# CloudResolvingClimateModeling/sp-coupler

Measured on AMD Instinct MI355X. Metric: SP column-exchanges/sec (GCM<->LES forcing+tendency), higher is better.
Workload: dtype f64

## Files before the change

include/spc.h:

```cpp
#ifndef SPC_H
#define SPC_H

#include <stdint.h>

#ifdef __cplusplus
extern "C" {
#endif

#define SPC_ABI_VERSION 4

typedef enum spc_status {
    SPC_OK = 0,
    SPC_ERR_INVALID_ARGUMENT = -1,
    SPC_ERR_UNSUPPORTED = -2,
    SPC_ERR_LAUNCH = -3,
    SPC_ERR_NO_DEVICE = -4
} spc_status;

typedef struct spc_dims {
    int64_t n_cols;
    int32_t nG;
    int32_t nL;
    int64_t pitchG;
    int64_t pitchGh;
    int64_t pitchL;
    int32_t les_grid_shared;
    int32_t cols_per_block;
} spc_dims;

typedef struct spc_forward_args {
    const void *U, *V, *T, *SH, *QL, *QI, *Pf;
    const void *Ph;
    const void *Zgfull;
    const void *Zghalf;
    const void *zf;
    const void *zh;
    const void *u_d, *v_d, *thl_d, *qt_d, *ql_d;
    const void *ps_d;
    const void *rain, *rain_last;
    double factor;
    double dt;
    void *f_u, *f_v, *f_thl, *f_qt, *f_ql, *ql_ref;
    void *f_ps;
    void *u, *v, *thl, *qt;
    void *ps;
    void *Zf;
    void *Zh;
    void *rainrate;
    int32_t *idx;
    const void *Z0M, *Z0H, *QLflux, *QIflux, *SHflux, *TSflux;
    void *z0m, *z0h, *wthl, *wqt;
} spc_forward_args;

int spc_forward_f64(const spc_dims *dims, const spc_forward_args *args, void *stream);
int spc_forward_f32(const spc_dims *dims, const spc_forward_args *args, void *stream);

int spc_cloud_indices_f64(const spc_dims *dims, const void *zh, const void *Zh, int32_t *idx, void *stream);
int spc_cloud_indices_f32(const spc_dims *dims, const void *zh, const void *Zh, int32_t *idx, void *stream);

typedef struct spc_backward_args {
    const void *T, *SH, *QL, *QI, *U, *V, *A;
    const void *Zf;
    const void *Zgfull, *Zghalf;
    const void *zf;
    const void *t_d, *qt_d, *ql_d, *ql_ice_d, *u_d, *v_d;
    const void *A_prof;
    const void *zh;
    const void *Zh;
    const void *rhobf_d;
    int32_t conservative;
    int32_t reserved;
    double factor;
    double dt;
    void *f_T, *f_SH, *f_QL, *f_QI, *f_U, *f_V, *f_A;
    int32_t *start_index;
} spc_backward_args;

int spc_backward_f64(const spc_dims *dims, const spc_backward_args *args, void *stream);
int spc_backward_f32(const spc_dims *dims, const spc_backward_args *args, void *stream);

typedef struct spc_diagnostics_args {
    const void *T, *SH, *QL, *QI, *Pf;
    const void *Zgfull, *Zghalf;
    const void *zf;
    const void *thl_d, *ql_d, *ql_ice_d;
    void *Tv, *THL, *QT;
    void *Zf;
    void *Zh;
    void *pf, *t, *ql_water;
} spc_diagnostics_args;

int spc_diagnostics_f64(const spc_dims *dims, const spc_diagnostics_args *args, void *stream);
int spc_diagnostics_f32(const spc_dims *dims, const spc_diagnostics_args *args, void *stream);

int spc_surface_fluxes_f64(int64_t n, const void *Ph_s, const void *T_s, const void *QLflux, const void *QIflux,
                           const void *SHflux, const void *TSflux, void *wthl, void *wqt, void *stream);
int spc_surface_fluxes_f32(int64_t n, const void *Ph_s, const void *T_s, const void *QLflux, const void *QIflux,
                           const void *SHflux, const void *TSflux, void *wthl, void *wqt, void *stream);

typedef struct spc_vnudge_args {
    int64_t n_cols;
    int32_t itot, jtot, ktot;
    int32_t constantT;
    void *qt;
// ... 179 lines not shown
```

sp_coupler_amd/_abi.py:

```python
import ctypes
import os

ABI_VERSION = 4
_HERE = os.path.dirname(os.path.abspath(__file__))
LIB_NAME = "libspc_hip.so"
LIB_PATH = os.path.join(_HERE, LIB_NAME)

c_void_p, c_double, c_int32, c_int64 = ctypes.c_void_p, ctypes.c_double, ctypes.c_int32, ctypes.c_int64
c_int32_p = ctypes.POINTER(ctypes.c_int32)

SPC_OK, SPC_ERR_INVALID_ARGUMENT, SPC_ERR_UNSUPPORTED, SPC_ERR_LAUNCH, SPC_ERR_NO_DEVICE = 0, -1, -2, -3, -4


class SpcError(RuntimeError):

    def __init__(self, code, text):
        super().__init__("spc error %d: %s" % (code, text))
        self.code = code


class SpcInvalidArgument(SpcError, ValueError):
    pass


class SpcLibraryError(ImportError):
    """The HIP extension is missing or does not match include/spc.h."""


class Dims(ctypes.Structure):
    _fields_ = [("n_cols", c_int64), ("nG", c_int32), ("nL", c_int32), ("pitchG", c_int64),
                ("pitchGh", c_int64), ("pitchL", c_int64), ("les_grid_shared", c_int32),
                ("cols_per_block", c_int32)]


def _ptrs(*names):
    return [(n, c_void_p) for n in names]


class ForwardArgs(ctypes.Structure):
    _fields_ = (_ptrs("U", "V", "T", "SH", "QL", "QI", "Pf", "Ph", "Zgfull", "Zghalf", "zf", "zh",
                      "u_d", "v_d", "thl_d", "qt_d", "ql_d", "ps_d", "rain", "rain_last")
                + [("factor", c_double), ("dt", c_double)]
                + _ptrs("f_u", "f_v", "f_thl", "f_qt", "f_ql", "ql_ref", "f_ps", "u", "v", "thl", "qt", "ps",
                        "Zf", "Zh", "rainrate", "idx", "Z0M", "Z0H", "QLflux", "QIflux", "SHflux", "TSflux",
                        "z0m", "z0h", "wthl", "wqt"))


class BackwardArgs(ctypes.Structure):
    _fields_ = (_ptrs("T", "SH", "QL", "QI", "U", "V", "A", "Zf", "Zgfull", "Zghalf", "zf",
                      "t_d", "qt_d", "ql_d", "ql_ice_d", "u_d", "v_d", "A_prof", "zh", "Zh", "rhobf_d")
                + [("conservative", c_int32), ("reserved", c_int32), ("factor", c_double), ("dt", c_double)]
                + _ptrs("f_T", "f_SH", "f_QL", "f_QI", "f_U", "f_V", "f_A", "start_index"))


class DiagnosticsArgs(ctypes.Structure):
    _fields_ = _ptrs("T", "SH", "QL", "QI", "Pf", "Zgfull", "Zghalf", "zf", "thl_d", "ql_d", "ql_ice_d",
                     "Tv", "THL", "QT", "Zf", "Zh", "pf", "t", "ql_water")


class VnudgeArgs(ctypes.Structure):
    _fields_ = ([("n_cols", c_int64), ("itot", c_int32), ("jtot", c_int32), ("ktot", c_int32), ("constantT", c_int32)]
                + _ptrs("qt", "qsat", "thl", "ql", "R", "ql_av", "qt_av", "presf", "ql_ref", "beta", "a_add", "qt_std", "status", "work")
                + [("work_bytes", c_int64)])


class InterpArgs(ctypes.Structure):
    _fields_ = ([("n_rows", c_int64), ("n_x", c_int32), ("n_xp", c_int32), ("pitch_x", c_int64), ("pitch_xp", c_int64),
                 ("pitch_fp", c_int64), ("pitch_out", c_int64)] + _ptrs("x", "xp", "fp", "out"))


class SearchsortedArgs(ctypes.Structure):
    _fields_ = ([("n_rows", c_int64), ("n_a", c_int32), ("n_v", c_int32), ("pitch_a", c_int64), ("pitch_v", c_int64),
                 ("pitch_out", c_int64)] + _ptrs("a", "v", "out") + [("side_right", c_int32), ("reserved", c_int32)])


class InterpCArgs(ctypes.Structure):
    _fields_ = ([("n_rows", c_int64), ("nG", c_int32), ("nL", c_int32), ("pitch_Zh", c_int64), ("pitch_zh", c_int64),
                 ("pitch_q", c_int64), ("pitch_out", c_int64)] + _ptrs("Zh", "zh", "q", "rho", "out")
                + [("mode", c_int32), ("reserved", c_int32)])


class PipArgs(ctypes.Structure):
    _fields_ = ([("n_points", c_int64), ("n_vertices", c_int64), ("n_rings", c_int32), ("n_polys", c_int32)]
                + _ptrs("lon", "lat", "vx", "vy", "ring_start", "ring_role", "ring_poly", "out"))


class LesStateArgs(ctypes.Structure):
    _fields_ = ([("n_les", c_int64)] + _ptrs("elem_off", "ktot") + [("prof", c_void_p * 4), ("pitch_prof", c_int64),
                ("amp", c_double * 4), ("out", c_void_p * 4)] + _ptrs("key_in") + [("pos_in", c_int32), ("reserved", c_int32)]
                + _ptrs("key_out", "pos_out") + [("gens_per_substream", c_int64)] + _ptrs("work") + [("work_bytes", c_int64)])


SLAB_MAX_FIELDS = 16


class SlabMeansArgs(ctypes.Structure):
    _fields_ = [("n_les", c_int64), ("itot", c_int32), ("jtot", c_int32), ("ktot", c_int32), ("n_fields", c_int32),
                ("fields", c_void_p * SLAB_MAX_FIELDS), ("out", c_void_p * SLAB_MAX_FIELDS), ("pitch_out", c_int64)]
# ... 152 lines not shown
```

sp_coupler_amd/csrc/spc_device.hpp:

```cpp
#pragma once

constexpr int BLOCK = 256;
constexpr int MAX_LDS_BYTES = 64 * 1024;
constexpr int HARD_LDS_BYTES = 160 * 1024;

template <typename T> struct K {
    static constexpr T pref0 = T(1e5), rd = T(287.04), rv = T(461.5), cp = T(1004.), rlv = T(2.53e6),
                       grav = T(9.81);
};

#define SPC_POW_FN __device__ __forceinline__
#include "spc_pow.h"
__device__ __forceinline__ double spc_pow_special(double x, double y)
{
    if (x != x) return x;
    const double big = __builtin_huge_val();
    if (x == 0.0) return y < 0.0 ? big : 0.0;
    if (x == big || x == -big) return y < 0.0 ? 0.0 : big;
    return __builtin_nan("");
}
__device__ __forceinline__ double spc_pow(double x, double y)
{
    if (!(x > 0.0 && x <= 1.7976931348623157e308)) return spc_pow_special(x, y);
    return spc_pow_pos(x, y);
// ... 209 lines not shown
    while (lo < hi) {
        const int mid = lo + ((hi - lo) >> 1);
        if (z[mid] < a) lo = mid + 1; else hi = mid;
    }
    return lo - 1;
}

__host__ __device__ inline int su_pad(int p2) { return 2 * p2 + 2; }

template <int SL, typename T, typename Pred> __device__ __forceinline__ const T *su_seek(const T *row, int p2, const Pred &adv)
{
    const T *p = row;
    if constexpr (SL > 0) {
#pragma unroll
        for (int s = 1 << (SL - 1); s > 0; s >>= 1) {
            const T *const nx = p + s;
            p = adv(p[s - 1]) ? nx : p;
        }
    } else {
        for (int s = p2; s > 0; s >>= 1) {
            const T *const nx = p + s;
            p = adv(p[s - 1]) ? nx : p;
        }
    }
    return p;
}

template <int SL, typename T, typename Pred> __device__ __forceinline__ int su_count(const T *row, int p2, const Pred &adv)
{
    return (int)(((unsigned)(size_t)su_seek<SL>(row, p2, adv) - (unsigned)(size_t)row) / (unsigned)sizeof(T));
}

struct DimsP {
    int64_t n_cols, pitchG, pitchGh, pitchL;
    int nG, nL, cb, p2G, p2L, shared_grid, xcd_remap;
};

struct Empty {};

template <typename T> struct FwdOpt {
    const T *rain, *rain_last;
    T *u, *v, *thl, *qt, *ps, *Zf, *Zh, *rainrate;
    const T *Z0M, *Z0H, *QLflux, *QIflux, *SHflux, *TSflux;
    T *z0m, *z0h, *wthl, *wqt;
};

template <typename T, bool FULL> struct FwdP {
    DimsP d;
    const T *U, *V, *Tm, *SH, *QL, *QI, *Pf, *Ph, *Zgfull, *Zghalf, *zf, *zh;
    const T *u_d, *v_d, *thl_d, *qt_d, *ql_d, *ps_d;
    T factor, dt;
    T *f_u, *f_v, *f_thl, *f_qt, *f_ql, *ql_ref, *f_ps;
    int32_t *idx;
    typename std::conditional<FULL, FwdOpt<T>, Empty>::type o;
};

template <typename T> using FwdFull = FwdP<T, true>;

template <typename T> struct BwdP {
    DimsP d;
    const T *Tm, *SH, *QL, *QI, *U, *V, *A, *Zf, *Zgfull, *Zghalf, *zf;
    const T *t_d, *qt_d, *ql_d, *ql_ice_d, *u_d, *v_d, *A_prof;
    const T *zh, *Zh, *rhobf_d;
    T factor, dt;
    T *f_T, *f_SH, *f_QL, *f_QI, *f_U, *f_V, *f_A;
    int32_t *start_index;
};

template <typename T> struct DiagP {
    DimsP d;
    const T *Tm, *SH, *QL, *QI, *Pf, *Zgfull, *Zghalf, *zf, *thl_d, *ql_d, *ql_ice_d;
    T *Tv, *THL, *QT, *Zf, *Zh, *pf, *t, *ql_water;
};

extern __shared__ __align__(16) unsigned char spc_smem[];

__device__ __forceinline__ unsigned slab_index(int remap)
{
    if (remap) {
        const unsigned b = blockIdx.x, nb = gridDim.x, x = b & 7u, j = b >> 3, q = nb >> 3, r = nb & 7u;
        return x * q + (x < r ? x : r) + j;
    }
    return blockIdx.x;
}

#ifdef SPC_STAMPS
__device__ unsigned long long *g_stamps = nullptr;
#define STAMP(i)                                                                     \
    do {                                                                             \
        if (threadIdx.x == 0 && g_stamps && (SPC_STAMPS == 1 || (i) == 0 || (i) == 5)) {  \
            asm volatile("s_waitcnt vmcnt(0) lgkmcnt(0)" ::: "memory");              \
            g_stamps[(size_t)blockIdx.x * 8 + (i)] = wall_clock64();                 \
        }                                                                            \
    } while (0)
#else
#define STAMP(i) do { } while (0)
#endif
```

sp_coupler_amd/csrc/spc_k1.hpp:

```cpp
#pragma once

template <typename T> struct LesIn {
    T h, ud, vd, thld, qtd, qld;
};

template <typename P, typename T = decltype(+*P().zf)>
__device__ __forceinline__ LesIn<T> load_les(const P &p, int l, int64_t o)
{
    LesIn<T> r;
    r.h = p.d.shared_grid ? ldg(&p.zf[l]) : ldg(&p.zf[o]);
    r.ud = ldg(&p.u_d[o]); r.vd = ldg(&p.v_d[o]); r.thld = ldg(&p.thl_d[o]); r.qtd = ldg(&p.qt_d[o]); r.qld = ldg(&p.ql_d[o]);
    return r;
}

constexpr int cfloor_pow2(int n) { int p = 1; while (p * 2 <= n) p *= 2; return p; }

template <typename T, bool FULL, int NG, int NL, int WT, int BLK = BLOCK, bool PRE = true>
__global__ __launch_bounds__(BLK) void k_forward(const FwdP<T, FULL> p)
{
    const DimsP &d = p.d;
#define OPT(f) (*(decltype(FwdOpt<T>::f) const volatile __attribute__((address_space(4))) *)( \
    (const char __attribute__((address_space(4))) *)__builtin_amdgcn_kernarg_segment_ptr() + offsetof(FwdFull<T>, o) + offsetof(FwdOpt<T>, f)))
    const int nG = NG ? NG : d.nG, nL = NL ? NL : d.nL, cb = d.cb;
    const int64_t pitchG = NG ? NG : d.pitchG, pitchGh = NG ? NG + 1 : d.pitchGh, pitchL = NL ? NL : d.pitchL;
    const int p2G = NG ? cfloor_pow2(NG ? NG : 1) : d.p2G;
    const int tid = threadIdx.x;
    const int64_t col0 = (int64_t)slab_index(d.xcd_remap) * cb;
    const int ncol = (int)((d.n_cols - col0) < cb ? (d.n_cols - col0) : cb);
    T *const lds = reinterpret_cast<T *>(spc_smem);
    T *const lzh = lds + (size_t)cb * 6 * nG;
    const int n1 = ncol * nG, n2 = ncol * nL, nI = p.idx ? n1 : 0, nitems = n2 + nI;
    constexpr bool REACH = !PRE;
    STAMP(0);

    LesIn<T> pre2 = {};
    T pre_zgh = T(0), pre_zs = T(0);
    if (!PRE) {
    } else if (tid < n2) {
        const int c = tid / nL, l = tid - c * nL;
        pre2 = load_les<FwdP<T, FULL>, T>(p, l, (col0 + c) * pitchL + l);
    } else if (tid < nitems) {
        const int ei = tid - n2, c = ei / nG, m = ei - c * nG;
        const int64_t gh = (col0 + c) * pitchGh;
        pre_zgh = ldg(&p.Zghalf[gh + (nG - 1 - m)]);
        pre_zs = ldg(&p.Zghalf[gh + nG]);
    }
    const int sc = BLK - 1 - tid;
    T sc_ps = T(0), sc_psd = T(0), sc_rain = T(0), sc_rl = T(0);
    if (PRE && sc < ncol) {
        sc_ps = ldg(&p.Ph[(col0 + sc) * pitchGh + nG]);
        sc_psd = ldg(&p.ps_d[col0 + sc]);
        if constexpr (FULL)
            if (OPT(rainrate)) { sc_rain = OPT(rain)[col0 + sc]; sc_rl = OPT(rain_last)[col0 + sc]; }
    }
    if (p.idx) {
        const int nz = d.shared_grid ? nL : n2;
        for (int e = tid; e < nz; e += BLK) {
            const int c = e / nL, l = e - c * nL;
            lzh[e] = d.shared_grid ? p.zh[e] : p.zh[(col0 + c) * pitchL + l];
        }
    }
    STAMP(1);

    int nR = nG;
    if constexpr (REACH) {
        __shared__ T s_wmax[BLK / 64];
        __shared__ int s_top;
        if (tid == 0) s_top = 0;
        for (int e = tid; e < n1; e += BLK) {
            const int c = e / nG, k = e - c * nG;
            const int64_t col = col0 + c, g = col * pitchG + k;
            const T zf_k = div_grav(ldg(&p.Zgfull[g]) - ldg(&p.Zghalf[col * pitchGh + nG]));
            lds[(size_t)c * 6 * nG + (nG - 1 - k)] = zf_k;
            if constexpr (FULL)
                if (OPT(Zf)) OPT(Zf)[g] = zf_k;
        }
        T hmax = T(-__builtin_huge_val());
        for (int e = tid, nz = d.shared_grid ? nL : n2; e < nz; e += BLK) {
            const int c = e / nL, l = e - c * nL;
            const T h = d.shared_grid ? ldg(&p.zf[e]) : ldg(&p.zf[(col0 + c) * pitchL + l]);
            hmax = h > hmax ? h : hmax;
        }
        for (int m = 32; m > 0; m >>= 1) {
            const T o = __shfl_xor(hmax, m, 64);
            hmax = o > hmax ? o : hmax;
        }
        if ((tid & 63) == 0) s_wmax[tid >> 6] = hmax;
        __syncthreads();
        if (tid < ncol) {
            for (int w = 0; w < BLK / 64; ++w) hmax = s_wmax[w] > hmax ? s_wmax[w] : hmax;
            const Br<T> b = bracket2(lds + (size_t)tid * 6 * nG, nG, p2G, hmax);
            atomicMax(&s_top, b.j0 + 1 >= nG ? nG - 1 : b.j0 + 1);
        }
        __syncthreads();
        nR = s_top + 1;
    }
    const float rcp_nR = 1.0f / (float)nR;
    for (int e = tid; e < ncol * nR; e += BLK) {
        int c, k;
        if constexpr (REACH) {
            c = (int)((float)e * rcp_nR);
            int r = e - c * nR;
            if (r < 0) { --c; r += nR; } else if (r >= nR) { ++c; r -= nR; }
            k = nG - nR + r;
        } else {
            c = e / nG; k = e - c * nG;
        }
        const int64_t col = col0 + c, g = col * pitchG + k;
        const T zsurf = REACH ? T(0) : ldg(&p.Zghalf[col * pitchGh + nG]);
        const T tt = ldg(&p.Tm[g]), sh = ldg(&p.SH[g]), ql = ldg(&p.QL[g]), qi = ldg(&p.QI[g]), pf = ldg(&p.Pf[g]);
        const T zg = REACH ? T(0) : ldg(&p.Zgfull[g]);
        const T uu = ldg(&p.U[g]), vv = ldg(&p.V[g]);
        T *const s = lds + (size_t)c * 6 * nG + (nG - 1 - k);
        if constexpr (!REACH) {
            const T zf_k = div_grav(zg - zsurf);
            s[0] = zf_k;
            if constexpr (FULL)
                if (OPT(Zf)) OPT(Zf)[g] = zf_k;
        }
        s[2 * nG] = sh + ql + qi;
        s[3 * nG] = ql;
        s[4 * nG] = uu;
        s[5 * nG] = vv;
        const T iex = spc_pow(div_pref0(pf), (-K<T>::rd) / K<T>::cp);
        s[nG] = (tt - div_cp(K<T>::rlv * (ql + qi))) * iex;
    }
    STAMP(2);
    __syncthreads();
    STAMP(3);

    if (sc < ncol) {
        const int64_t col = col0 + sc;
        if (!PRE) {
            sc_ps = ldg(&p.Ph[col * pitchGh + nG]); sc_psd = ldg(&p.ps_d[col]);
            if constexpr (FULL)
                if (OPT(rainrate)) { sc_rain = OPT(rain)[col]; sc_rl = OPT(rain_last)[col]; }
        }
        stg<WT>(&p.f_ps[col], Divisor<T>(p.dt).div(p.factor * (sc_ps - sc_psd)));
        if constexpr (FULL) {
            if (OPT(ps)) OPT(ps)[col] = sc_ps;
            if (OPT(rainrate)) OPT(rainrate)[col] = (sc_rain - sc_rl) / p.dt;
            if (OPT(wthl)) {
                const T rho = sc_ps / (K<T>::rd * ldg(&p.Tm[col * pitchG + (nG - 1)]));
                OPT(wqt)[col] = -(OPT(QLflux)[col] + OPT(QIflux)[col] + OPT(SHflux)[col]) / rho;
                OPT(wthl)[col] = -OPT(TSflux)[col] * spc_pow(div_pref0(sc_ps), (-K<T>::rd) / K<T>::cp)
                                / (K<T>::cp * rho);
                if (OPT(z0m)) OPT(z0m)[col] = OPT(Z0M)[col];
                if (OPT(z0h)) OPT(z0h)[col] = OPT(Z0H)[col];
            }
        }
    }

    const Divisor<T> ddt(p.dt);
    for (int e = tid; e < nitems; e += BLK) {
        if (e < n2) {
            const int c = e / nL, l = e - c * nL;
            const int64_t col = col0 + c, o = col * pitchL + l;
            const T *const s = lds + (size_t)c * 6 * nG;
            const LesIn<T> in = (PRE && e == tid) ? pre2 : load_les<FwdP<T, FULL>, T>(p, l, o);
            const Br<T> b = bracket2(s, nG, p2G, in.h);
            T f0[5], f1[5], r[5];
#pragma unroll
            for (int k = 0; k < 5; ++k) {
                f0[k] = s[(k + 1) * nG + b.j0];
                f1[k] = s[(k + 1) * nG + b.j1];
            }
            interp_fields<5>(b, f0, f1, r);
            const T thl = r[0], qt = r[1], ql = r[2], u = r[3], v = r[4];
            stg<WT>(&p.f_u[o], ddt.div(p.factor * (u - in.ud)));
            stg<WT>(&p.f_v[o], ddt.div(p.factor * (v - in.vd)));
            stg<WT>(&p.f_thl[o], ddt.div(p.factor * (thl - in.thld)));
            stg<WT>(&p.f_qt[o], ddt.div(p.factor * (qt - in.qtd)));
            stg<WT>(&p.f_ql[o], ddt.div(p.factor * (ql - in.qld)));
            stg<WT>(&p.ql_ref[o], ql);
            if constexpr (FULL) {
                if (OPT(u)) OPT(u)[o] = u;
                if (OPT(v)) OPT(v)[o] = v;
                if (OPT(thl)) OPT(thl)[o] = thl;
                if (OPT(qt)) OPT(qt)[o] = qt;
            }
        } else {
            const int ei = e - n2, c = ei / nG, m = ei - c * nG;
            const int64_t col = col0 + c, gh = col * pitchGh;
            const T zgh = (PRE && e == tid) ? pre_zgh : ldg(&p.Zghalf[gh + (nG - 1 - m)]);
            const T zs = (PRE && e == tid) ? pre_zs : ldg(&p.Zghalf[gh + nG]);
            const T Zh_k = div_grav(zgh - zs);
            const T *const zh = d.shared_grid ? lzh : lzh + (size_t)c * nL;
            p.idx[col * pitchG + m] = ss_right(zh, nL, Zh_k);
        }
    }
    STAMP(4);

    if constexpr (FULL) {
        if (OPT(Zh)) {
            for (int e = tid; e < ncol * (nG + 1); e += BLK) {
                const int c = e / (nG + 1), k = e - c * (nG + 1);
                const int64_t gh = (col0 + c) * pitchGh;
                OPT(Zh)[gh + k] = div_grav(ldg(&p.Zghalf[gh + k]) - ldg(&p.Zghalf[gh + nG]));
            }
        }
    }
    STAMP(5);
#undef OPT
}

template <typename T>
__global__ __launch_bounds__(BLOCK) void k_cloud_idx(const DimsP d, const T *zh_, const T *Zh_, int32_t *idx)
{
    const int nG = d.nG, nL = d.nL, cb = d.cb, tid = threadIdx.x;
    const int64_t col0 = (int64_t)slab_index(d.xcd_remap) * cb;
    const int ncol = (int)((d.n_cols - col0) < cb ? (d.n_cols - col0) : cb);
    T *const lzh = reinterpret_cast<T *>(spc_smem);
    const int nz = d.shared_grid ? nL : ncol * nL;
    for (int e = tid; e < nz; e += BLOCK) {
        const int c = e / nL, l = e - c * nL;
        lzh[e] = d.shared_grid ? zh_[e] : zh_[(col0 + c) * d.pitchL + l];
    }
    __syncthreads();
    for (int e = tid; e < ncol * nG; e += BLOCK) {
        const int c = e / nG, m = e - c * nG;
        const int64_t col = col0 + c;
        const T *const zh = d.shared_grid ? lzh : lzh + (size_t)c * nL;
        idx[col * d.pitchG + m] = ss_right(zh, nL, Zh_[col * d.pitchGh + (nG - 1 - m)]);
    }
}
```

sp_coupler_amd/csrc/spc_launch.hpp:

```cpp
#pragma once

thread_local char g_err[512] = "";

int fail(int code, const char *fmt, const char *a = "", long long b = 0, long long c = 0)
{
    snprintf(g_err, sizeof(g_err), fmt, a, b, c);
    return code;
}

int env_int(const char *name, int dflt)
{
    const char *e = getenv(name);
    return e ? atoi(e) : dflt;
}

int device_cus()
{
    const int forced = env_int("SPC_CUS", 0);
    if (forced > 0) return forced;
    thread_local int cache[64] = {0};
    int dev = 0;
    if (hipGetDevice(&dev) != hipSuccess) {
        (void)hipGetLastError();
        return 256;
// ... 221 lines not shown
    else
        c->cb = sb ? sb : pick_cb(d, 0, with_idx, sizeof(T), fwd_lean_kernel<T>(c->geo, 0, BLOCK, c->pre));
    c->vec = std::is_same<T, float>::value && c->geo != 0 && !full && !sb && !c->pre && c->cb % 2 == 0 && env_int("SPC_F32_VEC", 1);
    return choose_shape<T>(d, 0, with_idx, c);
}

inline KLean<float> fwd_vec_kernel(int geo, int wt)
{
    static const KLean<float> k[2][4] = {{nullptr, k_forward_f32v<91, 160, 0>, k_forward_f32v<137, 512, 0>, k_forward_f32v<19, 160, 0>},
                                         {nullptr, k_forward_f32v<91, 160, 1>, k_forward_f32v<137, 512, 1>, k_forward_f32v<19, 160, 1>}};
    return k[wt ? 1 : 0][geo];
}
inline bool aligned8(std::initializer_list<const void *> ptrs)
{
    for (const void *q : ptrs) if ((uintptr_t)q & 7u) return false;
    return true;
}

template <typename T> int forward_impl(const spc_dims *d, const spc_forward_args *a, void *stream)
{
    int rc = validate(d);
    if (rc) return rc;
    if (!a) return fail(SPC_ERR_INVALID_ARGUMENT, "%sargs is NULL");
    if (d->n_cols == 0) return SPC_OK;
    REQUIRE(a->U, "U"); REQUIRE(a->V, "V"); REQUIRE(a->T, "T"); REQUIRE(a->SH, "SH"); REQUIRE(a->QL, "QL");
    REQUIRE(a->QI, "QI"); REQUIRE(a->Pf, "Pf"); REQUIRE(a->Ph, "Ph"); REQUIRE(a->Zgfull, "Zgfull");
    REQUIRE(a->Zghalf, "Zghalf"); REQUIRE(a->zf, "zf"); REQUIRE(a->u_d, "u_d"); REQUIRE(a->v_d, "v_d");
    REQUIRE(a->thl_d, "thl_d"); REQUIRE(a->qt_d, "qt_d"); REQUIRE(a->ql_d, "ql_d"); REQUIRE(a->ps_d, "ps_d");
    REQUIRE(a->f_u, "f_u"); REQUIRE(a->f_v, "f_v"); REQUIRE(a->f_thl, "f_thl"); REQUIRE(a->f_qt, "f_qt");
    REQUIRE(a->f_ql, "f_ql"); REQUIRE(a->ql_ref, "ql_ref"); REQUIRE(a->f_ps, "f_ps");
    if (a->idx && !a->zh) return fail(SPC_ERR_INVALID_ARGUMENT, "%sidx requested but zh is NULL");
    if (a->rainrate && (!a->rain || !a->rain_last))
        return fail(SPC_ERR_INVALID_ARGUMENT, "%srainrate requested but rain / rain_last is NULL");
    if (a->wthl || a->wqt) {
        if (!a->wthl || !a->wqt || !a->QLflux || !a->QIflux || !a->SHflux || !a->TSflux)
            return fail(SPC_ERR_INVALID_ARGUMENT, "%ssurface coupling needs wthl, wqt and QLflux,QIflux,SHflux,TSflux");
        if ((a->z0m && !a->Z0M) || (a->z0h && !a->Z0H))
            return fail(SPC_ERR_INVALID_ARGUMENT, "%sz0m/z0h requested but Z0M/Z0H is NULL");
    }
    const bool with_idx = a->idx != nullptr;
    const bool full = a->u || a->v || a->thl || a->qt || a->ps || a->Zf || a->Zh || a->rainrate || a->wthl;
    Choice c;
    if ((rc = choose_fwd<T>(d, with_idx, full, &c))) return rc;
#define CP(f) p.f = (const T *)a->f
#define OP(f) p.f = (T *)a->f
#define COP(f) p.o.f = (const T *)a->f
#define OOP(f) p.o.f = (T *)a->f
    auto fill = [&](auto &p) {
        p.d = make_dims(d, c.cb);
        CP(U); CP(V); p.Tm = (const T *)a->T; CP(SH); CP(QL); CP(QI); CP(Pf); CP(Ph); CP(Zgfull); CP(Zghalf);
        CP(zf); CP(zh); CP(u_d); CP(v_d); CP(thl_d); CP(qt_d); CP(ql_d); CP(ps_d);
        p.factor = (T)a->factor; p.dt = (T)a->dt;
        OP(f_u); OP(f_v); OP(f_thl); OP(f_qt); OP(f_ql); OP(ql_ref); OP(f_ps); p.idx = a->idx;
    };
    if (full) {
        const KFull<T> kern = fwd_full_kernel<T>(c.geo, c.pre);
        FwdP<T, true> p;
        fill(p);
        COP(rain); COP(rain_last); OOP(u); OOP(v); OOP(thl); OOP(qt); OOP(ps); OOP(Zf); OOP(Zh); OOP(rainrate);
        COP(Z0M); COP(Z0H); COP(QLflux); COP(QIflux); COP(SHflux); COP(TSflux); OOP(z0m); OOP(z0h); OOP(wthl); OOP(wqt);
        return launch(kern, c, stream, "forward", p);
    } else {
        KLean<T> kern = fwd_lean_kernel<T>(c.geo, c.wt, c.blk, c.pre);
        if constexpr (std::is_same<T, float>::value) {
            if (c.vec && aligned8({a->U, a->V, a->T, a->SH, a->QL, a->QI, a->Pf, a->Zgfull, a->zf, a->u_d, a->v_d, a->thl_d, a->qt_d, a->ql_d,
                                   a->f_u, a->f_v, a->f_thl, a->f_qt, a->f_ql, a->ql_ref}))
                kern = fwd_vec_kernel(c.geo, c.wt);
        }
        if (!kern) return fail(SPC_ERR_UNSUPPORTED, "%sforward: no kernel instantiated for this launch choice (internal)");
        FwdP<T, false> p;
        fill(p);
        return launch(kern, c, stream, "forward", p);
    }
}

template <typename T> int choose_idx(const spc_dims *d, Choice *c)
{
    c->kernel = "k_cloud_idx"; c->elem = (int)sizeof(T); c->full = c->idx = c->geo = c->wt = c->pre = 0;
    c->blk = BLOCK;
    c->cb = pick_cb(d, 2, true, sizeof(T), k_cloud_idx<T>);
    return choose_shape<T>(d, 2, true, c);
}

template <typename T>
int cloud_idx_impl(const spc_dims *d, const void *zh, const void *Zh, int32_t *idx, void *stream)
{
    int rc = validate(d);
    if (rc) return rc;
    if (d->n_cols == 0) return SPC_OK;
    REQUIRE(zh, "zh"); REQUIRE(Zh, "Zh"); REQUIRE(idx, "idx");
    Choice c;
    if ((rc = choose_idx<T>(d, &c))) return rc;
    return launch(k_cloud_idx<T>, c, stream, "cloud_indices", make_dims(d, c.cb), (const T *)zh, (const T *)Zh, idx);
}

#define SPC_BWD_ROW(WT_, BLK_, PRE_)                                                                                 \
    {k_backward<T, 0, 0, WT_, BLK_, PRE_>, k_backward<T, 91, 160, WT_, BLK_, PRE_>, k_backward<T, 137, 512, WT_, BLK_, PRE_>, \
     k_backward<T, 19, 160, WT_, BLK_, PRE_>}
#define SPC_BWD_ROW_BIG(BLK_)                                                                                        \
    {k_backward<T, 0, 0, 1, BLK_, true>, k_backward<T, 91, 160, 1, BLK_, true>, nullptr, k_backward<T, 19, 160, 1, BLK_, true>}

template <typename T> KBwd<T> bwd_kernel(int geo, int wt, int blk, int pre)
{
    static const KBwd<T> k256[2][2][4] = {{SPC_BWD_ROW(0, BLOCK, false), SPC_BWD_ROW(1, BLOCK, false)},
                                          {SPC_BWD_ROW(0, BLOCK, true), SPC_BWD_ROW(1, BLOCK, true)}};
    static const KBwd<T> k512[4] = SPC_BWD_ROW_BIG(512), k1024[4] = SPC_BWD_ROW_BIG(1024);
// ... 207 lines not shown
```

sp_coupler_amd/engine.py:

```python
import contextlib
import ctypes

import torch

from . import _abi

SURF_IN = ("Z0M", "Z0H", "QLflux", "QIflux", "SHflux", "TSflux")
FWD_LES = ("U", "V", "THL", "QT", "QL")
BWD_LES = ("T", "QT", "QL", "QL_ice", "U", "V")

_DTYPES = {torch.float64: "f64", torch.float32: "f32"}
LES_STATE_FIELDS = ("U", "V", "THL", "QT")
LES_STATE_AMPS = (0.5, 0.5, 0.1, 2.5e-5)


def _stream_ptr(stream, device=None):
    if stream is None:
        stream = torch.cuda.current_stream(device)
    elif device is not None and stream.device != device:
        raise ValueError("stream is on %s, engine is on %s" % (stream.device, device))
    return ctypes.c_void_p(stream.cuda_stream)


def _on_engine_stream(fn):
# ... 29 lines not shown
        if t.dim() != 2 or t.shape[0] != n or t.shape[1] != m:
            raise ValueError("%s must have shape [%d x %d], got %s" % (name, n, m, tuple(t.shape)))
        if m > 1 and t.stride(1) != 1:
            raise ValueError("%s must be contiguous along levels (stride %s)" % (name, t.stride()))
        p = t.stride(0) if n > 1 else (pitch if pitch is not None else max(m, t.stride(0)))
        if pitch is not None and n > 1 and p != pitch:
            raise ValueError("%s has column pitch %d, batch uses %d" % (name, p, pitch))
        if p < m:
            raise ValueError("%s has column pitch %d < %d levels" % (name, p, m))
        self.keep.append(t)
        return t.data_ptr(), p

    def vec(self, name, t, n, dtype=None):
        if not isinstance(t, torch.Tensor):
            raise TypeError("%s must be a torch.Tensor, got %s" % (name, type(t).__name__))
        if t.device != self.device or t.dtype != (dtype or self.dtype):
            raise ValueError("%s must be %s on %s" % (name, dtype or self.dtype, self.device))
        if t.dim() != 1 or t.shape[0] != n or (n > 1 and t.stride(0) != 1):
            raise ValueError("%s must be a contiguous vector of %d, got %s" % (name, n, tuple(t.shape)))
        self.keep.append(t)
        return t.data_ptr()


class _Plan:

    def __init__(self, engine, fn, call_args, keep, outputs, dims=None, args=None):
        self.engine, self._fn, self._call, self._keep, self.outputs = engine, fn, tuple(call_args), keep, outputs
        self.dims, self.args = dims, args

    def set_scalars(self, factor, dt):
        self.args.factor, self.args.dt = float(factor), float(dt)

    def launch(self, stream=None):
        eng = self.engine
        if stream is None:
            stream = eng.stream
        with torch.cuda.device(eng.device):
            rc = self._fn(*self._call, _stream_ptr(stream, eng.device))
        if rc:
            _abi.check(eng.lib, rc)
        return self.outputs

    def launch_raw(self, stream_ptr):
        rc = self._fn(*self._call, stream_ptr)
        if rc:
            _abi.check(self.engine.lib, rc)

    def describe(self):
        return _abi.describe_launch(self.engine.lib, self.dims, self._pass, self._flags(), 8 if self.engine.dtype == torch.float64 else 4)


class ForwardPlan(_Plan):
    _pass = 0

    def _flags(self):
        a = self.args
        full = any(getattr(a, f) for f in ("u", "v", "thl", "qt", "ps", "Zf", "Zh", "rainrate", "wthl"))
        return (1 if a.idx else 0) | (2 if full else 0)


class BackwardPlan(_Plan):
    @property
    def _pass(self):
        return 4 if self.args.conservative else 1

    def _flags(self):
        return 0


class DiagnosticsPlan(_Plan):
    _pass = 3

    def _flags(self):
        return 0


class CloudIndexPlan(_Plan):
    _pass = 2

    def _flags(self):
        return 0


class SurfacePlan(_Plan):
    def describe(self):
        return "k_surface"


class OperatorPlan(_Plan):

    def __init__(self, engine, fn, call_args, keep, outputs, result, refresh=()):
        super().__init__(engine, fn, call_args, keep, outputs)
        self.result = result
        self._refresh = tuple(refresh)

    def run(self, stream=None):
        if self._refresh:
            eng = self.engine
            st = stream if stream is not None else eng.stream
            with (torch.cuda.stream(st) if st is not None else contextlib.nullcontext()):
                for snap, src in self._refresh:
                    snap.copy_(src if src.shape == snap.shape else src.expand_as(snap))
        self.launch(stream)
        return self.result

    def launch_raw(self, stream_ptr):
# ... 5 lines not shown
    def describe(self):
        return getattr(self._fn, "__name__", "operator")


class Engine:

    def __init__(self, device=None, dtype=torch.float64, stream=None, lib_path=None):
        self.stream = stream
        self.lib = _abi.load_library(lib_path)
        if dtype not in _DTYPES:
            raise ValueError("dtype must be torch.float64 or torch.float32")
        if not torch.cuda.is_available() or self.lib.spc_device_count() < 1:
            raise RuntimeError("sp_coupler_amd.Engine needs a HIP device (MI355X); there is no CPU fallback")
        self.device = torch.device(device if device is not None else "cuda:%d" % torch.cuda.current_device())
        if self.device.type != "cuda":
            raise ValueError("Engine device must be a cuda/HIP device")
        if self.device.index is None:
            self.device = torch.device("cuda", torch.cuda.current_device())
        self.dtype = dtype
        sfx = _DTYPES[dtype]
        self._vn_work = None
        self._es_tab = None
        self._fwd = getattr(self.lib, "spc_forward_" + sfx)
        self._bwd = getattr(self.lib, "spc_backward_" + sfx)
        self._idx = getattr(self.lib, "spc_cloud_indices_" + sfx)
        self._diag = getattr(self.lib, "spc_diagnostics_" + sfx)

    def _grid(self, ck, name, z, n, nL, pitchL):
        if z.dim() == 1:
            return ck.vec(name, z, nL), 1
        ptr, _ = ck.mat(name, z, n, nL, pitchL)
        return ptr, 0

    def empty(self, *shape, dtype=None):
        return torch.empty(*shape, device=self.device, dtype=dtype or self.dtype)

    def on_stream(self):
        return torch.cuda.stream(self.stream) if self.stream is not None else contextlib.nullcontext()

    def synchronize(self):
        (self.stream if self.stream is not None else torch.cuda.current_stream(self.device)).synchronize()

    def arena(self, specs, rows=None):
        from .transfer import Arena
        return Arena(self.device, specs, stream=self.stream)

    def to_devices(self, host_array, rows=None, n_cols=None, dtype=None):
        import numpy
        with self.on_stream():
            return torch.from_numpy(numpy.ascontiguousarray(host_array)).to(self.device, dtype or self.dtype)

    @_on_engine_stream
    def plan_forward(self, gcm, zf, prof, factor, dt, zh=None, *, want_profiles=False, want_heights=True,
                     want_idx=None, couple_surface=False, cols_per_block=0, out=None):
        T_ = gcm["T"]
        n, nG = int(T_.shape[0]), int(T_.shape[1])
        nL = int(prof["U"].shape[1])
        ck = _Checker(self.device, self.dtype)
        a = _abi.ForwardArgs()
        pitchG = pitchGh = pitchL = None
        for key, field in (("U", "U"), ("V", "V"), ("T", "T"), ("SH", "SH"), ("QL", "QL"), ("QI", "QI"),
                           ("Pfull", "Pf"), ("Zgfull", "Zgfull")):
            ptr, pitchG = ck.mat("gcm[%s]" % key, gcm[key], n, nG, pitchG)
            setattr(a, field, ptr)
        for key, field in (("Phalf", "Ph"), ("Zghalf", "Zghalf")):
            ptr, pitchGh = ck.mat("gcm[%s]" % key, gcm[key], n, nG + 1, pitchGh)
            setattr(a, field, ptr)
        for key, field in zip(FWD_LES, ("u_d", "v_d", "thl_d", "qt_d", "ql_d")):
            ptr, pitchL = ck.mat("prof[%s]" % key, prof[key], n, nL, pitchL)
            setattr(a, field, ptr)
        a.ps_d = ck.vec("prof[PS]", prof["PS"], n)
        a.zf, shared = self._grid(ck, "zf", zf, n, nL, pitchL)
        if want_idx is None:
            want_idx = zh is not None
        out = dict(out or {})
        res = {}

        def omat(name, m, pitch):
            t = out.get(name)
            if t is None:
                t = torch.empty(n, pitch or m, device=self.device, dtype=self.dtype)[:, :m]
            ptr, _ = ck.mat("out[%s]" % name, t, n, m, pitch)
            res[name] = t
            return ptr

        def ovec(name):
            t = out.get(name)
            if t is None:
                t = self.empty(n)
            res[name] = t
            return ck.vec("out[%s]" % name, t, n)

        for name in ("f_u", "f_v", "f_thl", "f_qt", "f_ql", "ql_ref"):
            setattr(a, name, omat(name, nL, pitchL))
        a.f_ps = ovec("f_ps")
        if want_profiles:
            for name in ("u", "v", "thl", "qt"):
                setattr(a, name, omat(name, nL, pitchL))
            a.ps = ovec("ps")
        if want_heights:
            a.Zf = omat("Zf", nG, pitchG)
            a.Zh = omat("Zh", nG + 1, pitchGh)
        if want_idx:
            if zh is None:
                raise ValueError("want_idx needs the LES half-level heights zh")
            a.zh, sh2 = self._grid(ck, "zh", zh, n, nL, pitchL)
            if sh2 != shared:
                raise ValueError("zf and zh must both be shared [nL] or both per column [n x nL]")
            idx = out.get("idx")
            if idx is None:
                idx = torch.empty(n, pitchG or nG, device=self.device, dtype=torch.int32)[:, :nG]
            if (idx.dtype != torch.int32 or idx.device != self.device or tuple(idx.shape) != (n, nG)
                    or (nG > 1 and idx.stride(1) != 1) or (n > 1 and idx.stride(0) != pitchG)):
                raise ValueError("out[idx] must be int32 [%d x %d] with column pitch %d" % (n, nG, pitchG))
            ck.keep.append(idx)
            a.idx = idx.data_ptr()
            res["idx"] = idx
        if "Rain" in prof and "rain_last" in prof:
            a.rain = ck.vec("prof[Rain]", prof["Rain"], n)
            a.rain_last = ck.vec("prof[rain_last]", prof["rain_last"], n)
            a.rainrate = ovec("rainrate")
        if couple_surface:
            for key in SURF_IN:
                setattr(a, key, ck.vec("gcm[%s]" % key, gcm[key], n))
            for name in ("z0m", "z0h", "wthl", "wqt"):
                setattr(a, name, ovec(name))
        a.factor, a.dt = float(factor), float(dt)
        dims = _abi.Dims(n, nG, nL, pitchG or nG, pitchGh or nG + 1, pitchL or nL, shared, int(cols_per_block))
        return ForwardPlan(self, self._fwd, (ctypes.byref(dims), ctypes.byref(a)), ck.keep, res, dims, a)

    @_on_engine_stream
    def forward(self, *args, stream=None, **kw):
        return self.plan_forward(*args, **kw).launch(stream)

    @_on_engine_stream
    def plan_cloud_indices(self, zh, Zh, out=None, cols_per_block=0):
        n, nGp1 = int(Zh.shape[0]), int(Zh.shape[1])
        nG = nGp1 - 1
        nL = int(zh.shape[-1])
        ck = _Checker(self.device, self.dtype)
        Zh_ptr, pitchGh = ck.mat("Zh", Zh, n, nG + 1)
        zh_ptr, shared = self._grid(ck, "zh", zh, n, nL, None)
        pitchL = zh.stride(0) if (zh.dim() == 2 and n > 1) else nL
        idx = out if out is not None else self.empty(n, nG, dtype=torch.int32)
        if (idx.dtype != torch.int32 or idx.device != self.device or tuple(idx.shape) != (n, nG)
                or (nG > 1 and idx.stride(1) != 1)):
            raise ValueError("out must be int32 [%d x %d] on %s, contiguous along levels" % (n, nG, self.device))
        pitchI = idx.stride(0) if n > 1 else nG
        ck.keep.append(idx)
        dims = _abi.Dims(n, nG, nL, pitchI, pitchGh, pitchL, shared, int(cols_per_block))
        return CloudIndexPlan(self, self._idx, (ctypes.byref(dims), zh_ptr, Zh_ptr, idx.data_ptr()), ck.keep, {"idx": idx}, dims)

    @_on_engine_stream
    def cloud_indices(self, zh, Zh, stream=None, cols_per_block=0):
        return self.plan_cloud_indices(zh, Zh, cols_per_block=cols_per_block).launch(stream)["idx"]

    @_on_engine_stream
    def plan_backward(self, gcm, zf, prof, factor, dt, Zf=None, *, want_start_index=True, conservative=False,
                      zh=None, Zh=None, cols_per_block=0, out=None):
        T_ = gcm["T"]
        n, nG = int(T_.shape[0]), int(T_.shape[1])
        nL = int(prof["T"].shape[1])
        ck = _Checker(self.device, self.dtype)
        a = _abi.BackwardArgs()
        pitchG = pitchGh = pitchL = None
        for key in ("T", "SH", "QL", "QI", "U", "V", "A"):
            ptr, pitchG = ck.mat("gcm[%s]" % key, gcm[key], n, nG, pitchG)
            setattr(a, key, ptr)
        if Zf is not None:
            a.Zf, pitchG = ck.mat("Zf", Zf, n, nG, pitchG)
        else:
            a.Zgfull, pitchG = ck.mat("gcm[Zgfull]", gcm["Zgfull"], n, nG, pitchG)
            a.Zghalf, pitchGh = ck.mat("gcm[Zghalf]", gcm["Zghalf"], n, nG + 1, pitchGh)
        for key, field in zip(BWD_LES, ("t_d", "qt_d", "ql_d", "ql_ice_d", "u_d", "v_d")):
            ptr, pitchL = ck.mat("prof[%s]" % key, prof[key], n, nL, pitchL)
            setattr(a, field, ptr)
        a.A_prof, pitchG = ck.mat("prof[A]", prof["A"], n, nG, pitchG)
        a.zf, shared = self._grid(ck, "zf", zf, n, nL, pitchL)
        a.conservative = 1 if conservative else 0
        if conservative:
            if zh is None:
                raise ValueError("conservative coarsening needs the LES half-level heights zh")
            a.zh, sh2 = self._grid(ck, "zh", zh, n, nL, pitchL)
            if sh2 != shared:
                raise ValueError("zf and zh must both be shared [nL] or both per column [n x nL]")
# ... 525 lines not shown
```

Baseline: 130.9 million.

## Speculatively preload forward reach levels using a persistent device-side hint

Adds a device-resident reach hint that keeps the maximum reached level count from earlier launches. The forward kernel uses it to issue GCM field loads for those top levels before the wave max reduction and bracket search finish, then loads only the levels beyond the hint. The aim is to overlap global-memory latency with the reduction and search phase instead of serialising them. It also reads several kernel arguments directly from the kernarg segment. The cost is extra shared state, an atomic max per block, and wasted loads if the hint overestimates the needed levels.

```diff
diff --git a/include/spc.h b/include/spc.h
--- a/include/spc.h
+++ b/include/spc.h
@@ -50,6 +50,7 @@
     int32_t *idx;
     const void *Z0M, *Z0H, *QLflux, *QIflux, *SHflux, *TSflux;
     void *z0m, *z0h, *wthl, *wqt;
+    int32_t *reach_hint;
 } spc_forward_args;
 
 int spc_forward_f64(const spc_dims *dims, const spc_forward_args *args, void *stream);
diff --git a/sp_coupler_amd/_abi.py b/sp_coupler_amd/_abi.py
--- a/sp_coupler_amd/_abi.py
+++ b/sp_coupler_amd/_abi.py
@@ -43,7 +43,7 @@
                 + [("factor", c_double), ("dt", c_double)]
                 + _ptrs("f_u", "f_v", "f_thl", "f_qt", "f_ql", "ql_ref", "f_ps", "u", "v", "thl", "qt", "ps",
                         "Zf", "Zh", "rainrate", "idx", "Z0M", "Z0H", "QLflux", "QIflux", "SHflux", "TSflux",
-                        "z0m", "z0h", "wthl", "wqt"))
+                        "z0m", "z0h", "wthl", "wqt", "reach_hint"))
 
 
 class BackwardArgs(ctypes.Structure):
diff --git a/sp_coupler_amd/csrc/spc_device.hpp b/sp_coupler_amd/csrc/spc_device.hpp
--- a/sp_coupler_amd/csrc/spc_device.hpp
+++ b/sp_coupler_amd/csrc/spc_device.hpp
@@ -285,6 +285,7 @@
     T factor, dt;
     T *f_u, *f_v, *f_thl, *f_qt, *f_ql, *ql_ref, *f_ps;
     int32_t *idx;
+    int32_t *reach_hint;
     typename std::conditional<FULL, FwdOpt<T>, Empty>::type o;
 };
 
diff --git a/sp_coupler_amd/csrc/spc_k1.hpp b/sp_coupler_amd/csrc/spc_k1.hpp
--- a/sp_coupler_amd/csrc/spc_k1.hpp
+++ b/sp_coupler_amd/csrc/spc_k1.hpp
@@ -13,6 +13,39 @@
     return r;
 }
 
+template <typename T> struct FwdIn {
+    T tt, sh, ql, qi, pf, uu, vv;
+};
+
+template <typename T> struct FwdPtr {
+    const T *Tm, *SH, *QL, *QI, *Pf, *U, *V;
+};
+
+template <typename T> __device__ __forceinline__ FwdIn<T> load_fwd(const FwdPtr<T> &p, int64_t g)
+{
+    FwdIn<T> r;
+    r.tt = ldg(&p.Tm[g]); r.sh = ldg(&p.SH[g]); r.ql = ldg(&p.QL[g]); r.qi = ldg(&p.QI[g]); r.pf = ldg(&p.Pf[g]);
+    r.uu = ldg(&p.U[g]); r.vv = ldg(&p.V[g]);
+    return r;
+}
+
+template <typename T> __device__ __forceinline__ void stage_fwd(T *s, int nG, const FwdIn<T> &in)
+{
+    s[2 * nG] = in.sh + in.ql + in.qi;
+    s[3 * nG] = in.ql;
+    s[4 * nG] = in.uu;
+    s[5 * nG] = in.vv;
+    const T iex = spc_pow(div_pref0(in.pf), (-K<T>::rd) / K<T>::cp);
+    s[nG] = (in.tt - div_cp(K<T>::rlv * (in.ql + in.qi))) * iex;
+}
+
+__device__ __forceinline__ void split_rt(int e, int n, float rcp_n, int &c, int &r)
+{
+    c = (int)((float)e * rcp_n);
+    r = e - c * n;
+    if (r < 0) { --c; r += n; } else if (r >= n) { ++c; r -= n; }
+}
+
 constexpr int cfloor_pow2(int n) { int p = 1; while (p * 2 <= n) p *= 2; return p; }
 
 template <typename T, bool FULL, int NG, int NL, int WT, int BLK = BLOCK, bool PRE = true>
@@ -21,6 +54,12 @@
     const DimsP &d = p.d;
 #define OPT(f) (*(decltype(FwdOpt<T>::f) const volatile __attribute__((address_space(4))) *)( \
     (const char __attribute__((address_space(4))) *)__builtin_amdgcn_kernarg_segment_ptr() + offsetof(FwdFull<T>, o) + offsetof(FwdOpt<T>, f)))
+    using Params = FwdP<T, FULL>;
+#define KARG(f) (*(decltype(Params::f) const volatile __attribute__((address_space(4))) *)( \
+    (const char __attribute__((address_space(4))) *)__builtin_amdgcn_kernarg_segment_ptr() + offsetof(Params, f)))
+#define FIELD_PTRS() FwdPtr<T>{KARG(Tm), KARG(SH), KARG(QL), KARG(QI), KARG(Pf), KARG(U), KARG(V)}
+#define HINT_PTR (*(int32_t *const volatile __attribute__((address_space(4))) *)( \
+    (const char __attribute__((address_space(4))) *)__builtin_amdgcn_kernarg_segment_ptr() + offsetof(Params, reach_hint)))
     const int nG = NG ? NG : d.nG, nL = NL ? NL : d.nL, cb = d.cb;
     const int64_t pitchG = NG ? NG : d.pitchG, pitchGh = NG ? NG + 1 : d.pitchGh, pitchL = NL ? NL : d.pitchL;
     const int p2G = NG ? cfloor_pow2(NG ? NG : 1) : d.p2G;
@@ -31,6 +70,9 @@
     T *const lzh = lds + (size_t)cb * 6 * nG;
     const int n1 = ncol * nG, n2 = ncol * nL, nI = p.idx ? n1 : 0, nitems = n2 + nI;
     constexpr bool REACH = !PRE;
+    int hint = 0;
+    if constexpr (REACH)
+        if (int32_t *const q = HINT_PTR) hint = *q;
     STAMP(0);
 
     LesIn<T> pre2 = {};
@@ -62,11 +104,25 @@
     }
     STAMP(1);
 
-    int nR = nG;
+    int nR = nG, k0 = 0;
     if constexpr (REACH) {
         __shared__ T s_wmax[BLK / 64];
+        __shared__ int s_whint[BLK / 64];
         __shared__ int s_top;
         if (tid == 0) s_top = 0;
+        const int h = __builtin_amdgcn_readfirstlane(hint);
+        const int nH = h < 0 ? 0 : (h > nG ? nG : h);
+        const int nE = ncol * nH;
+        const float rcp_nH = 1.0f / (float)nH;
+        FwdIn<T> g0 = {};
+        T *s0 = lds;
+        if (tid < nE) {
+            int c, r;
+            split_rt(tid, nH, rcp_nH, c, r);
+            const int k = nG - nH + r;
+            g0 = load_fwd(FIELD_PTRS(), (col0 + c) * pitchG + k);
+            s0 = lds + (size_t)c * 6 * nG + (nG - 1 - k);
+        }
         for (int e = tid; e < n1; e += BLK) {
             const int c = e / nG, k = e - c * nG;
             const int64_t col = col0 + c, g = col * pitchG + k;
@@ -85,32 +141,49 @@
             const T o = __shfl_xor(hmax, m, 64);
             hmax = o > hmax ? o : hmax;
         }
-        if ((tid & 63) == 0) s_wmax[tid >> 6] = hmax;
+        if ((tid & 63) == 0) { s_wmax[tid >> 6] = hmax; s_whint[tid >> 6] = nH; }
+        if (tid < nE) stage_fwd(s0, nG, g0);
+        if (tid + BLK < nE) {
+            const FwdPtr<T> fp = FIELD_PTRS();
+        for (int e = tid + BLK; e < nE; e += BLK) {
+            int c, r;
+            split_rt(e, nH, rcp_nH, c, r);
+            const int k = nG - nH + r;
+            const FwdIn<T> in = load_fwd(fp, (col0 + c) * pitchG + k);
+            stage_fwd(lds + (size_t)c * 6 * nG + (nG - 1 - k), nG, in);
+        }
+        }
         __syncthreads();
         if (tid < ncol) {
-            for (int w = 0; w < BLK / 64; ++w) hmax = s_wmax[w] > hmax ? s_wmax[w] : hmax;
+            hmax = s_wmax[0];
+            for (int w = 1; w < BLK / 64; ++w) hmax = s_wmax[w] > hmax ? s_wmax[w] : hmax;
             const Br<T> b = bracket2(lds + (size_t)tid * 6 * nG, nG, p2G, hmax);
             atomicMax(&s_top, b.j0 + 1 >= nG ? nG - 1 : b.j0 + 1);
         }
+        int nV = s_whint[0];
+        for (int w = 1; w < BLK / 64; ++w) nV = s_whint[w] == nV ? nV : 0;
         __syncthreads();
-        nR = s_top + 1;
+        const int top1 = s_top + 1;
+        nR = top1 > nV ? top1 - nV : 0;
+        k0 = nG - top1;
+        if (nR > 0 && tid == 0)
+            if (int32_t *const q = HINT_PTR) __hip_atomic_fetch_max(q, top1, __ATOMIC_RELAXED, __HIP_MEMORY_SCOPE_AGENT);
     }
     const float rcp_nR = 1.0f / (float)nR;
+    const FwdPtr<T> fp = REACH ? FIELD_PTRS() : FwdPtr<T>{p.Tm, p.SH, p.QL, p.QI, p.Pf, p.U, p.V};
     for (int e = tid; e < ncol * nR; e += BLK) {
         int c, k;
         if constexpr (REACH) {
-            c = (int)((float)e * rcp_nR);
-            int r = e - c * nR;
-            if (r < 0) { --c; r += nR; } else if (r >= nR) { ++c; r -= nR; }
-            k = nG - nR + r;
+            split_rt(e, nR, rcp_nR, c, k);
+            k += k0;
         } else {
             c = e / nG; k = e - c * nG;
         }
         const int64_t col = col0 + c, g = col * pitchG + k;
         const T zsurf = REACH ? T(0) : ldg(&p.Zghalf[col * pitchGh + nG]);
-        const T tt = ldg(&p.Tm[g]), sh = ldg(&p.SH[g]), ql = ldg(&p.QL[g]), qi = ldg(&p.QI[g]), pf = ldg(&p.Pf[g]);
+        const T tt = ldg(&fp.Tm[g]), sh = ldg(&fp.SH[g]), ql = ldg(&fp.QL[g]), qi = ldg(&fp.QI[g]), pf = ldg(&fp.Pf[g]);
         const T zg = REACH ? T(0) : ldg(&p.Zgfull[g]);
-        const T uu = ldg(&p.U[g]), vv = ldg(&p.V[g]);
+        const T uu = ldg(&fp.U[g]), vv = ldg(&fp.V[g]);
         T *const s = lds + (size_t)c * 6 * nG + (nG - 1 - k);
         if constexpr (!REACH) {
             const T zf_k = div_grav(zg - zsurf);
@@ -129,14 +202,15 @@
     __syncthreads();
     STAMP(3);
 
+    T *const f_ps = REACH ? KARG(f_ps) : p.f_ps;
     if (sc < ncol) {
         const int64_t col = col0 + sc;
         if (!PRE) {
-            sc_ps = ldg(&p.Ph[col * pitchGh + nG]); sc_psd = ldg(&p.ps_d[col]);
+            sc_ps = ldg(&KARG(Ph)[col * pitchGh + nG]); sc_psd = ldg(&KARG(ps_d)[col]);
             if constexpr (FULL)
                 if (OPT(rainrate)) { sc_rain = OPT(rain)[col]; sc_rl = OPT(rain_last)[col]; }
         }
-        stg<WT>(&p.f_ps[col], Divisor<T>(p.dt).div(p.factor * (sc_ps - sc_psd)));
+        stg<WT>(&f_ps[col], Divisor<T>(p.dt).div(p.factor * (sc_ps - sc_psd)));
         if constexpr (FULL) {
             if (OPT(ps)) OPT(ps)[col] = sc_ps;
             if (OPT(rainrate)) OPT(rainrate)[col] = (sc_rain - sc_rl) / p.dt;
@@ -152,6 +226,7 @@
     }
 
     const Divisor<T> ddt(p.dt);
+    T *const f_u = REACH ? KARG(f_u) : p.f_u, *const f_v = REACH ? KARG(f_v) : p.f_v, *const f_thl = REACH ? KARG(f_thl) : p.f_thl;
     for (int e = tid; e < nitems; e += BLK) {
         if (e < n2) {
             const int c = e / nL, l = e - c * nL;
@@ -167,9 +242,9 @@
             }
             interp_fields<5>(b, f0, f1, r);
             const T thl = r[0], qt = r[1], ql = r[2], u = r[3], v = r[4];
-            stg<WT>(&p.f_u[o], ddt.div(p.factor * (u - in.ud)));
-            stg<WT>(&p.f_v[o], ddt.div(p.factor * (v - in.vd)));
-            stg<WT>(&p.f_thl[o], ddt.div(p.factor * (thl - in.thld)));
+            stg<WT>(&f_u[o], ddt.div(p.factor * (u - in.ud)));
+            stg<WT>(&f_v[o], ddt.div(p.factor * (v - in.vd)));
+            stg<WT>(&f_thl[o], ddt.div(p.factor * (thl - in.thld)));
             stg<WT>(&p.f_qt[o], ddt.div(p.factor * (qt - in.qtd)));
             stg<WT>(&p.f_ql[o], ddt.div(p.factor * (ql - in.qld)));
             stg<WT>(&p.ql_ref[o], ql);
@@ -202,6 +277,9 @@
     }
     STAMP(5);
 #undef OPT
+#undef HINT_PTR
+#undef FIELD_PTRS
+#undef KARG
 }
 
 template <typename T>
diff --git a/sp_coupler_amd/csrc/spc_launch.hpp b/sp_coupler_amd/csrc/spc_launch.hpp
--- a/sp_coupler_amd/csrc/spc_launch.hpp
+++ b/sp_coupler_amd/csrc/spc_launch.hpp
@@ -297,6 +297,7 @@
         CP(zf); CP(zh); CP(u_d); CP(v_d); CP(thl_d); CP(qt_d); CP(ql_d); CP(ps_d);
         p.factor = (T)a->factor; p.dt = (T)a->dt;
         OP(f_u); OP(f_v); OP(f_thl); OP(f_qt); OP(f_ql); OP(ql_ref); OP(f_ps); p.idx = a->idx;
+        p.reach_hint = a->reach_hint;
     };
     if (full) {
         const KFull<T> kern = fwd_full_kernel<T>(c.geo, c.pre);
diff --git a/sp_coupler_amd/engine.py b/sp_coupler_amd/engine.py
--- a/sp_coupler_amd/engine.py
+++ b/sp_coupler_amd/engine.py
@@ -105,6 +105,17 @@
 
 class ForwardPlan(_Plan):
     _pass = 0
+    _hint = None
+
+    @property
+    def reach_hint(self):
+        return self._hint
+
+    def reset_reach_hint(self):
+        if self._hint is not None:
+            st = self.engine.stream
+            with (torch.cuda.stream(st) if st is not None else contextlib.nullcontext()):
+                self._hint.zero_()
 
     def _flags(self):
         a = self.args
@@ -216,7 +227,7 @@
 
     @_on_engine_stream
     def plan_forward(self, gcm, zf, prof, factor, dt, zh=None, *, want_profiles=False, want_heights=True,
-                     want_idx=None, couple_surface=False, cols_per_block=0, out=None):
+                     want_idx=None, couple_surface=False, cols_per_block=0, out=None, reach_hint=True):
         T_ = gcm["T"]
         n, nG = int(T_.shape[0]), int(T_.shape[1])
         nL = int(prof["U"].shape[1])
@@ -290,11 +301,19 @@
             for name in ("z0m", "z0h", "wthl", "wqt"):
                 setattr(a, name, ovec(name))
         a.factor, a.dt = float(factor), float(dt)
+        hint = None
+        if reach_hint:
+            hint = torch.zeros(1, device=self.device, dtype=torch.int32)
+            ck.keep.append(hint)
+            a.reach_hint = hint.data_ptr()
         dims = _abi.Dims(n, nG, nL, pitchG or nG, pitchGh or nG + 1, pitchL or nL, shared, int(cols_per_block))
-        return ForwardPlan(self, self._fwd, (ctypes.byref(dims), ctypes.byref(a)), ck.keep, res, dims, a)
+        plan = ForwardPlan(self, self._fwd, (ctypes.byref(dims), ctypes.byref(a)), ck.keep, res, dims, a)
+        plan._hint = hint
+        return plan
 
     @_on_engine_stream
     def forward(self, *args, stream=None, **kw):
+        kw.setdefault("reach_hint", False)
         return self.plan_forward(*args, **kw).launch(stream)
 
     @_on_engine_stream
```

Result: no change. 130.8 million (-0.1%).
